# sidward14/gan-lab

Hardware: AMD Instinct MI355X
Metric: images/sec (G+D step), StyleGAN 1024^2 bs32/GPU (higher is better)
Workload: dtype f32; 1 GPU; StyleGAN res_samples=1024 FFHQ-shaped synthetic, bs=32/GPU fp32, nonsaturating + R1(lambda=10) + drift, stabilised phase, 1 D-iter + 1 G-iter; global_batch=32, per_gpu_batch=32, parallelism=single

## Files before the change

gan_lab_amd/_lib.py:

```python
import ctypes
import os
import subprocess

import torch

_HERE = os.path.dirname(os.path.abspath(__file__))
CSRC = os.path.join(_HERE, 'csrc')
SO_PATH = os.path.join(CSRC, os.path.basename(os.environ.get('GANLAB_HIP_LIB', '') or 'libganlab_hip.so'))

_c_int, _c_ll, _c_f, _c_p, _c_sz, _c_u64 = (ctypes.c_int, ctypes.c_longlong, ctypes.c_float, ctypes.c_void_p,
                                             ctypes.c_size_t, ctypes.c_uint64)

ACT_NONE, ACT_LRELU = 0, 1
PACK_FWD, PACK_DGRAD = 0, 1


class ConvGeom(ctypes.Structure):
    _fields_ = [('N', _c_int), ('Cin', _c_int), ('Hin', _c_int), ('Win', _c_int),
                ('Cout', _c_int), ('ks', _c_int), ('pad', _c_int), ('up', _c_int), ('pool', _c_int)]


_GP = ctypes.POINTER(ConvGeom)


# ... 49 lines not shown
    'ganlab_conv_s2_x3_pack': (_c_ll, [_c_p, _c_p, _c_int, _c_int, _c_int, _c_f, _c_p]),
    'ganlab_conv_s2_fwd_x3': (_c_int, [_c_p, _c_p, _c_p, _c_p, _GP, _c_f, _c_int, _c_f, _c_p]),
    'ganlab_conv_s2_fwd_aff_x3': (_c_int, [_c_p, _c_p, _c_p, _c_p, _c_p, _c_p, _GP, _c_f, _c_int, _c_f, _c_p]),
    'ganlab_conv_s2_dgrad_x3': (_c_int, [_c_p, _c_p, _c_p, _GP, _c_p]),
    'ganlab_conv_s2_down_x3_supported': (_c_int, [_GP, _c_int]),
    'ganlab_conv_s2_down_x3_pack': (_c_ll, [_c_p, _c_p, _c_int, _c_int, _c_int, _c_f, _c_p]),
    'ganlab_conv_s2_down_fwd_x3': (_c_int, [_c_p, _c_p, _c_p, _c_p, _GP, _c_f, _c_int, _c_f, _c_p]),
    'ganlab_conv_s2_down_dgrad_x3': (_c_int, [_c_p, _c_p, _c_p, _GP, _c_p]),
    'ganlab_conv_wgrad_x3_supported': (_c_int, [_GP]),
    'ganlab_conv_wgrad_x3_workspace': (_c_sz, [_GP]),
    'ganlab_conv_wgrad_x3': (_c_int, [_c_p, _c_p, _c_p, _c_p, _c_p, _GP, _c_f, _c_p, _c_sz, _c_p]),
    'ganlab_conv_s2_wgrad_x3_supported': (_c_int, [_GP]),
    'ganlab_conv_s2_wgrad_x3_workspace': (_c_sz, [_GP]),
    'ganlab_conv_s2_wgrad_x3': (_c_int, [_c_p, _c_p, _c_p, _c_p, _c_p, _GP, _c_f, _c_p, _c_sz, _c_p]),
    'ganlab_conv_fwd_aff_tail_x3': (_c_int, [_c_p, _c_p, _c_p, _c_p, _c_p, _c_p, _c_p, _c_p, _c_p, _c_p, _GP, _c_f, _c_int, _c_f,
                                             _c_f, _c_p, _c_sz, _c_p]),
    'ganlab_mask_bits_supported': (_c_int, [_c_int, _c_int]),
    'ganlab_blur3x3_bits_f32': (_c_int, [_c_p, _c_p, _c_p, _c_ll, _c_int, _c_int, _c_p]),
    'ganlab_blur_act_bwd_bits_f32': (_c_int, [_c_p, _c_p, _c_p, _c_p, _c_int, _c_int, _c_int, _c_int, _c_f, _c_f,
                                              _c_p, _c_sz, _c_p]),
    'ganlab_act_bwd_blur_bits_f32': (_c_int, [_c_p, _c_p, _c_p, _c_p, _c_p, _c_p, _c_int, _c_int, _c_int, _c_int,
                                              _c_f, _c_f, _c_p, _c_sz, _c_p]),
    'ganlab_conv_fwd_blur_supported': (_c_int, [_GP, _c_p, _c_p]),
    'ganlab_conv_fwd_blur_bits_f32': (_c_int, [_c_p, _c_p, _c_p, _c_p, _c_p, _GP, _c_f, _c_f, _c_p]),
    'ganlab_conv_s2_blur_supported': (_c_int, [_GP]),
    'ganlab_conv_s2_blur_workspace': (_c_sz, [_GP]),
    'ganlab_conv_s2_fwd_blur_tail_f32': (_c_int, [_c_p, _c_p, _c_p, _c_p, _c_p, _c_p, _c_p, _c_p, _c_p, _c_p, _GP, _c_f, _c_int,
                                                  _c_f, _c_f, _c_p, _c_sz, _c_p]),
    'ganlab_conv_s2_dgrad_blur_act_bits_f32': (_c_int, [_c_p, _c_p, _c_p, _c_p, _c_p, _GP, _c_f, _c_f, _c_p, _c_sz, _c_p]),
    'ganlab_conv_dgrad_rgb_sums_supported': (_c_int, [_GP, _c_int]),
    'ganlab_conv_dgrad_rgb_sums_workspace': (_c_sz, [_GP]),
    'ganlab_conv_dgrad_rgb_sums_f32': (_c_int, [_c_p, _c_p, _c_p, _c_p, _c_p, _c_p, _GP, _c_int, _c_f, _c_f, _c_f, _c_int, _c_int,
                                                _c_p, _c_sz, _c_p]),
    'ganlab_conv_fwd_bits_f32': (_c_int, [_c_p, _c_p, _c_p, _c_p, _c_p, _GP, _c_f, _c_int, _c_f, _c_p]),
    'ganlab_conv_dgrad_act_bits_f32': (_c_int, [_c_p, _c_p, _c_p, _c_p, _GP, _c_f, _c_p]),
    'ganlab_conv_fwd_mask_bits_f32': (_c_int, [_c_p, _c_p, _c_p, _c_p, _GP, _c_f, _c_p]),
    'ganlab_conv_wgrad_act_bits_f32': (_c_int, [_c_p, _c_p, _c_p, _c_p, _c_p, _GP, _c_f, _c_f, _c_f, _c_p, _c_sz, _c_p]),
    'ganlab_pack_desc_size': (_c_int, []),
    'ganlab_pack_many': (_c_int, [_c_p, _c_int, _c_ll, _c_p]),
    'ganlab_in_affine_f32': (_c_int, [_c_p, _c_p, _c_p, _c_p, _c_p, _c_int, _c_int, _c_p]),
    'ganlab_conv_aff_supported': (_c_int, [_GP]),
    'ganlab_conv_fwd_aff_f32': (_c_int, [_c_p, _c_p, _c_p, _c_p, _c_p, _c_p, _GP, _c_f, _c_int, _c_f, _c_p]),
    'ganlab_conv_fwd_aff_tail_chunks': (_c_int, [_GP]),
    'ganlab_conv_fwd_aff_tail_f32': (_c_int, [_c_p, _c_p, _c_p, _c_p, _c_p, _c_p, _c_p, _c_p, _c_p, _c_p, _GP, _c_f, _c_int, _c_f,
                                              _c_f, _c_p, _c_sz, _c_p]),
    'ganlab_conv_wgrad_aff_f32': (_c_int, [_c_p, _c_p, _c_p, _c_p, _c_p, _GP, _c_f, _c_p, _c_sz, _c_p]),
    'ganlab_conv_s2_aff_supported': (_c_int, [_GP]),
    'ganlab_conv_s2_fwd_aff_f32': (_c_int, [_c_p, _c_p, _c_p, _c_p, _c_p, _c_p, _GP, _c_f, _c_int, _c_f, _c_p]),
    'ganlab_conv_s2_wgrad_aff_f32': (_c_int, [_c_p, _c_p, _c_p, _c_p, _c_p, _GP, _c_f, _c_p, _c_sz, _c_p]),
    'ganlab_mod_conv_supported': (_c_int, [_GP]),
    'ganlab_mod_conv_stat_chunks': (_c_int, [_GP]),
    'ganlab_mod_conv_fwd_f32': (_c_int, [_c_p, _c_p, _c_p, _c_p, _c_p, _c_p, _c_p, _c_p, _c_p, _c_p, _GP, _c_f, _c_int,
                                         _c_f, _c_f, _c_p, _c_sz, _c_p]),
    'ganlab_mod_torgb_prep_f32': (_c_int, [_c_p, _c_p, _c_p, _c_p, _c_p, _c_p, _c_int, _c_int, _c_int, _c_f, _c_f, _c_p]),
    'ganlab_mod_torgb_wgrad_f32': (_c_int, [_c_p, _c_p, _c_p, _c_p, _c_p, _c_int, _c_int, _c_int, _c_f, _c_f, _c_p]),
    'ganlab_mod_torgb_fwd_f32': (_c_int, [_c_p, _c_p, _c_p, _c_p, _c_int, _c_int, _c_int, _c_ll, _c_p]),
    'ganlab_mod_torgb_cross_workspace': (_c_sz, [_c_int]),
    'ganlab_mod_torgb_cross_f32': (_c_int, [_c_p, _c_p, _c_p, _c_int, _c_int, _c_int, _c_ll, _c_p, _c_sz, _c_p]),
    'ganlab_blur3x3_f32': (_c_int, [_c_p, _c_p, _c_ll, _c_int, _c_int, _c_p]),
    'ganlab_up2_f32': (_c_int, [_c_p, _c_p, _c_ll, _c_int, _c_int, _c_f, _c_p]),
    'ganlab_pool2_f32': (_c_int, [_c_p, _c_p, _c_ll, _c_int, _c_int, _c_f, _c_p]),
    'ganlab_resample2d_f32': (_c_int, [_c_p, _c_p, _c_p, _c_p, _c_p, _c_p, _c_ll, _c_int, _c_int, _c_int, _c_int, _c_int,
                                       _c_int, _c_p]),
    'ganlab_bias_act_f32': (_c_int, [_c_p, _c_p, _c_p, _c_p, _c_p, _c_int, _c_int, _c_ll, _c_f, _c_int, _c_f, _c_p]),
    'ganlab_act_bwd_f32': (_c_int, [_c_p, _c_p, _c_p, _c_ll, _c_f, _c_p]),
    'ganlab_act_bwd_bias_f32': (_c_int, [_c_p, _c_p, _c_p, _c_p, _c_int, _c_int, _c_ll, _c_f, _c_f, _c_p, _c_sz, _c_p]),
# ... 152 lines not shown
```

gan_lab_amd/csrc/conv_roll_blur.hip:

```cpp
#include "common.h"

#include <stdlib.h>

namespace {

typedef unsigned int u32x4 __attribute__((ext_vector_type(4)));

constexpr int RB_TW = 64, RB_SLOTS = 6, RB_RP = 80, RB_SLOT = 16 * RB_RP, RB_Q = 18;
constexpr int RB_ITEMS = 4 * 16 * RB_Q;
constexpr int RB_PT = (RB_ITEMS + 255) / 256;
constexpr int RB_OOB = (int)0x80000000;
#ifndef RB_STORE_AUX
#define RB_STORE_AUX 0
#endif
#ifndef RB_LOAD_AUX
#define RB_LOAD_AUX 0
#endif
#ifndef RB_SETPRIO
#define RB_SETPRIO 0
#endif

struct RBArgs {
  const float* x;
  const float* wp;
  const float* bias;
  float* y;
  unsigned short* bits;
  int N, Cin, Cout, H, W;
  int Cin_p, Cout_p;
  int cols, strips, spu;
  float bias_scale, slope;
  int act;
  const float* img;
  const unsigned char* mbits;
  double* part;
  int img_c;
};
enum { RB_PLAIN = 0, RB_BLUR = 1, RB_RGB = 2 };

__device__ __forceinline__ float rb_act(float v, float slope) { return v > 0.f ? v : v * slope; }

#ifdef GL_PHASES
__device__ unsigned long long* rb_phase_buf;
#define RB_PH_DECL unsigned long long rb_t = wall_clock64(), rb_ph[10] = {0, 0, 0, 0, 0, 0, 0, 0, 0, 0};
#define RB_PH(i) { const unsigned long long rb_n = wall_clock64(); rb_ph[i] += rb_n - rb_t; rb_t = rb_n; }
#define RB_PH_FLUSH(nsteps) if (threadIdx.x == 0) { for (int i_ = 0; i_ < 10; ++i_) rb_phase_buf[(long long)blockIdx.x * 12 + i_] = rb_ph[i_]; \
    rb_phase_buf[(long long)blockIdx.x * 12 + 10] = (nsteps); rb_phase_buf[(long long)blockIdx.x * 12 + 11] = wall_clock64(); }
#else
#define RB_PH_DECL
#define RB_PH(i)
#define RB_PH_FLUSH(nsteps)
#endif

template <int MODE>
__global__ __launch_bounds__(256, MODE == RB_PLAIN ? 4 : 3) void conv_fwd_roll_blur_kernel(RBArgs p) {
  constexpr bool BLUR = MODE == RB_BLUR, RGB = MODE == RB_RGB;
  constexpr int RO = BLUR ? 1 : 0;
  __shared__ __attribute__((aligned(16))) float img_s[RGB ? 4 * 4 * 64 : 4];
  __shared__ double red_s[RGB ? 4 * 16 * 4 : 1];
  __shared__ __attribute__((aligned(16))) float ring[RB_SLOTS * RB_SLOT];
  __shared__ __attribute__((aligned(16))) float xn[2 * 4 * 16 * 4];
  __shared__ __attribute__((aligned(16))) float xe[2 * 4 * 16 * 4];
  __shared__ __attribute__((aligned(16))) unsigned bits_s[BLUR ? 16 * 8 : 4];
  __shared__ __attribute__((aligned(16))) float scratch_s[BLUR ? 256 * 4 : 4];
  const int tid = threadIdx.x, lane = tid & 63, w = tid >> 6;
  const int co = lane & 15, kk = lane >> 4;
  int bid = gl_xcd_remap(blockIdx.x, gridDim.x);
  const int txi = bid % p.cols;
  bid /= p.cols;
// ... 300 lines not shown
    }
    __syncthreads();
    if (kk == 0)
#pragma unroll
      for (int c = 0; c < 4; ++c) red_s[(w * 16 + co) * 4 + c] = rsum[c];
    __syncthreads();
    if (tid < 64 && (tid >> 2) < p.Cout) {
      const int c = tid & 3, ch = tid >> 2;
      const double t = (red_s[(0 * 16 + ch) * 4 + c] + red_s[(1 * 16 + ch) * 4 + c]) +
                       (red_s[(2 * 16 + ch) * 4 + c] + red_s[(3 * 16 + ch) * 4 + c]);
      p.part[(long long)(ch * 4 + c) * gridDim.x + blockIdx.x] = t;
    }
  }
}

__global__ void rb_rgb_finish_kernel(const double* __restrict__ part, float* __restrict__ gw, float* __restrict__ gb, int chunks,
                                     int img_c, float scale, float bias_scale, int accumulate) {
  const int ch = blockIdx.x >> 2, c = blockIdx.x & 3;
  double t = 0.0;
  for (int i = threadIdx.x; i < chunks; i += 64) t += part[(long long)blockIdx.x * chunks + i];
#pragma unroll
  for (int o = 32; o > 0; o >>= 1) t += __shfl_xor(t, o, 64);
  if (threadIdx.x != 0) return;
  if (c < img_c && gw != nullptr) {
    float* d = gw + ch * img_c + c;
    *d = ((accumulate & 1) ? *d : 0.f) + (float)(t * (double)scale);
  } else if (c == 3 && gb != nullptr) {
    gb[ch] = ((accumulate & 2) ? gb[ch] : 0.f) + (float)(t * (double)bias_scale);
  }
}

}

__global__ __launch_bounds__(256, 4) void conv_fwd_roll2_kernel(RBArgs p) {
  __shared__ __attribute__((aligned(16))) float ring[RB_SLOTS * RB_SLOT];
  constexpr int HITEMS = 2 * 16 * RB_Q, HPT = (HITEMS + 255) / 256;
  const int tid = threadIdx.x, lane = tid & 63, w = tid >> 6;
  const int co = lane & 15, kk = lane >> 4;
  int bid = gl_xcd_remap(blockIdx.x, gridDim.x);
  const int txi = bid % p.cols;
  bid /= p.cols;
  const int syi = bid % p.strips;
  const int n0 = bid / p.strips;
  const int nh = 2 * min(p.spu, p.H / 4 - syi * p.spu);
  const int ox0 = txi * RB_TW, Y0 = syi * p.spu * 4;
  const int plane = p.H * p.W;
  const float* xb = p.x + (long long)n0 * p.Cin * plane;

  int gb[HPT], lo[HPT];
#pragma unroll
  for (int i = 0; i < HPT; ++i) {
    const int e = tid + i * 256;
    const int q = e % RB_Q, t = e / RB_Q;
    const int ci = t & 15, k = t >> 4;
    const int vx = ox0 - 4 + 4 * q;
    gb[i] = (e < HITEMS && ci < p.Cin && (unsigned)vx < (unsigned)p.W) ? (ci * plane + vx) * 4 : RB_OOB;
    lo[i] = e < HITEMS ? ((ci * RB_RP + 4 * q) | (k << 16)) : -1;
  }
  float wreg[36];
#pragma unroll
  for (int st = 0; st < 36; ++st)
    wreg[st] = p.wp[(long long)((st >> 2) * p.Cin_p + (st & 3) * 4 + kk) * p.Cout_p + co];
  const bool co_ok = co < p.Cout;
  const float bv = (p.bias != nullptr && co_ok) ? p.bias[co] * p.bias_scale : 0.f;
  const long long oplane = (long long)p.H * p.W;
  const __amdgpu_buffer_rsrc_t rs_in =
      __builtin_amdgcn_make_buffer_rsrc(const_cast<float*>(xb), 0, (unsigned)(p.Cin * plane * 4), 0x00020000);
  const __amdgpu_buffer_rsrc_t rs_out = __builtin_amdgcn_make_buffer_rsrc(
      p.y + (long long)n0 * p.Cout * oplane, 0, (unsigned)(p.Cout * oplane * 4), 0x00020000);
  const int vo_lane = co_ok ? (int)(((long long)co * oplane + ox0 + w * 16 + kk * 4) * 4) : RB_OOB;
  const int W4 = p.W * 4;

  float4 xr[2][HPT];
  auto load_item = [&](int r0, bool on, int set, int i) {
    const int vy = Y0 - 1 + r0 + ((lo[i] >> 16) & 1);
    const int off = (on && gb[i] != RB_OOB && (unsigned)vy < (unsigned)p.H) ? gb[i] + vy * W4 : RB_OOB;
    const u32x4 v = __builtin_amdgcn_raw_buffer_load_b128(rs_in, off, 0, 0);
    xr[set][i] = float4{__uint_as_float(v.x), __uint_as_float(v.y), __uint_as_float(v.z), __uint_as_float(v.w)};
  };
  auto store_item = [&](int r0, int set, int i) {
    if (lo[i] != -1)
      *reinterpret_cast<float4*>(ring + ((r0 % RB_SLOTS) + ((lo[i] >> 16) & 1)) * RB_SLOT + (lo[i] & 0xffff)) = xr[set][i];
  };
#pragma unroll
  for (int i = 0; i < HPT; ++i) load_item(0, true, 0, i);
#pragma unroll
  for (int i = 0; i < HPT; ++i) load_item(2, true, 1, i);
#pragma unroll
  for (int i = 0; i < HPT; ++i) store_item(0, 0, i);
#pragma unroll
  for (int i = 0; i < HPT; ++i) store_item(2, 1, i);
#pragma unroll
  for (int i = 0; i < HPT; ++i) load_item(4, true, 0, i);
#pragma unroll
  for (int i = 0; i < HPT; ++i) load_item(6, nh > 2, 1, i);
  __syncthreads();

  f32x4 acc[2] = {f32x4{0.f, 0.f, 0.f, 0.f}, f32x4{0.f, 0.f, 0.f, 0.f}};
  const int a_lane = kk * RB_RP + w * 16 + co + 3;
  auto half_step = [&](int h, int par) {
    int sb[4];
#pragma unroll
    for (int j = 0; j < 4; ++j) sb[j] = ((2 * h + j) % RB_SLOTS) * RB_SLOT;
    constexpr int PD = 3, NF = 48;
    float rb[PD + 1];
    auto fj = [](int f) { return f < 24 ? (f & 1 ? 3 : 0) : (f < 36 ? 1 : 2); };
    auto fi = [](int f) { return f < 24 ? (f >> 1) : (f - 24) % 12; };
    auto fetch = [&](int f, int slot) {
      const int i12 = fi(f), kx = i12 >> 2, c4 = i12 & 3;
      rb[slot] = ring[sb[fj(f)] + c4 * 4 * RB_RP + kx + a_lane];
    };
    auto piece = [&](int k) {
      if (k < HPT) store_item(2 * h + 4, par, k);
      else load_item(2 * h + 8, h + 3 < nh, par, k - HPT);
    };
#pragma unroll
    for (int f = 0; f < PD; ++f) fetch(f, f % (PD + 1));
#pragma unroll
    for (int f = 0; f < NF; ++f) {
      if (f + PD < NF) fetch(f + PD, (f + PD) % (PD + 1));
      const int slot = f % (PD + 1), j = fj(f), i12 = fi(f), kx = i12 >> 2, c4 = i12 & 3;
#pragma unroll
      for (int r2 = 0; r2 < 2; ++r2) {
        const int ky = j - r2;
        if (ky >= 0 && ky < 3)
          acc[r2] = __builtin_amdgcn_mfma_f32_16x16x4f32(rb[slot], wreg[(ky * 3 + kx) * 4 + c4], acc[r2], 0, 0, 0);
      }
      if ((f & 7) == 3) {
        __builtin_amdgcn_sched_barrier(0);
        piece(f >> 3);
      }
      __builtin_amdgcn_sched_barrier(0);
    }
#pragma unroll
    for (int r2 = 0; r2 < 2; ++r2) {
      const int row = Y0 + 2 * h + r2;
      u32x4 o;
#pragma unroll
      for (int r = 0; r < 4; ++r) {
        float t = acc[r2][r] + bv;
        if (p.act == GANLAB_ACT_LRELU) t = gl_lrelu(t, p.slope);
        o[r] = __float_as_uint(t);
      }
      __builtin_amdgcn_raw_buffer_store_b128(o, rs_out, vo_lane == RB_OOB ? vo_lane : vo_lane + row * W4, 0, 0);
      acc[r2] = f32x4{0.f, 0.f, 0.f, 0.f};
    }
    __syncthreads();
  };
  for (int h = 0; h < nh; h += 2) {
    half_step(h, 0);
    half_step(h + 1, 1);
  }
}

static long long rb_plan(RBArgs& a, int N, int H, int W, int blur) {
  a.cols = W / RB_TW;
  const int steps = H / 4;
  const long long cols = (long long)a.cols * N;
  int k = 1;
  while (k < steps && cols * k < 4096 && (steps + k) / (k + 1) >= (blur ? 16 : 8)) ++k;
  a.spu = (steps + k - 1) / k;
  a.strips = (steps + a.spu - 1) / a.spu;
  return cols * a.strips;
}

bool gl_roll_blur_supported(int N, int Cin, int Cout, int H, int W, const void* x, const void* y) {
  return N > 0 && Cin >= 1 && Cin <= 16 && Cout >= 1 && Cout <= 16 && W % RB_TW == 0 && H % 4 == 0 &&
         (long long)Cin * H * W * 4 < 0x7fffffffLL && (long long)Cout * H * W * 4 < 0x7fffffffLL &&
         (reinterpret_cast<uintptr_t>(x) & 15) == 0 && (reinterpret_cast<uintptr_t>(y) & 15) == 0;
}

int gl_roll_blur_launch(const float* x, const float* wp, const float* bias, float* y, void* bits, int N, int Cin, int Cout,
                        int H, int W, int Cin_p, int Cout_p, float bias_scale, float slope, hipStream_t st, int blur,
                        int act) {
  RBArgs a{};
  a.x = x; a.wp = wp; a.bias = bias; a.y = y; a.bits = reinterpret_cast<unsigned short*>(bits);
  a.N = N; a.Cin = Cin; a.Cout = Cout; a.H = H; a.W = W; a.Cin_p = Cin_p; a.Cout_p = Cout_p;
  a.bias_scale = bias_scale; a.slope = slope; a.act = act;
  const long long grid = rb_plan(a, N, H, W, blur);
  if (grid <= 0 || grid > 0x7fffffffLL) return GANLAB_EINVAL;
  static const int half = [] { const char* e = getenv("GANLAB_ROLL_HALF"); return (e && e[0] == '0') ? 0 : 1; }();
  if (blur) GL_LAUNCH(conv_fwd_roll_blur_kernel<RB_BLUR>, dim3((unsigned)grid), dim3(256), 0, st, a);
  else if (half) GL_LAUNCH(conv_fwd_roll2_kernel, dim3((unsigned)grid), dim3(256), 0, st, a);
  else GL_LAUNCH(conv_fwd_roll_blur_kernel<RB_PLAIN>, dim3((unsigned)grid), dim3(256), 0, st, a);
  return GL_CHECK_LAUNCH();
// ... 27 lines not shown
}

size_t ganlab_conv_dgrad_rgb_sums_workspace(const ganlab_conv_geom* g) {
  if (!ganlab_conv_dgrad_rgb_sums_supported(g, 3)) return 0;
  RBArgs a{};
  const long long grid = rb_plan(a, g->N, g->Hin, g->Win, 0);
  return (size_t)g->Cin * 4 * (size_t)grid * sizeof(double);
}

int ganlab_conv_dgrad_rgb_sums_f32(const float* gy, const float* wp, const unsigned* ybits, const float* img, float* gw_rgb,
                                   float* gb_rgb, const ganlab_conv_geom* g, int img_c, float scale, float bias_scale,
                                   float slope, int acc_w, int acc_b, void* workspace, size_t workspace_bytes, void* stream) {
  if (!gy || !wp || !ybits || !img || !g || (!gw_rgb && !gb_rgb)) return GANLAB_EINVAL;
  if (!ganlab_conv_dgrad_rgb_sums_supported(g, img_c) || (reinterpret_cast<uintptr_t>(gy) & 15) ||
      (reinterpret_cast<uintptr_t>(img) & 15))
    return GANLAB_EUNSUPPORTED;
  if (!workspace || workspace_bytes < ganlab_conv_dgrad_rgb_sums_workspace(g)) return GANLAB_EWORKSPACE;
  RBArgs a{};
  a.x = gy; a.wp = wp; a.bias = nullptr; a.y = nullptr; a.bits = nullptr;
  a.N = g->N; a.Cin = g->Cout; a.Cout = g->Cin; a.H = g->Hin; a.W = g->Win;
  a.Cin_p = (g->Cout + 15) / 16 * 16; a.Cout_p = (g->Cin + 63) / 64 * 64;
  a.bias_scale = 0.f; a.slope = slope; a.act = GANLAB_ACT_NONE;
  a.img = img; a.mbits = reinterpret_cast<const unsigned char*>(ybits); a.part = reinterpret_cast<double*>(workspace);
  a.img_c = img_c;
  const long long grid = rb_plan(a, g->N, g->Hin, g->Win, 0);
  if (grid <= 0 || grid > 0x7fffffffLL) return GANLAB_EINVAL;
  hipStream_t st = gl_stream(stream);
  GL_LAUNCH(conv_fwd_roll_blur_kernel<RB_RGB>, dim3((unsigned)grid), dim3(256), 0, st, a);
  GL_LAUNCH(rb_rgb_finish_kernel, dim3((unsigned)(g->Cin * 4)), dim3(64), 0, st, (const double*)a.part, gw_rgb, gb_rgb,
            (int)grid, img_c, scale, bias_scale, (acc_w ? 1 : 0) | (acc_b ? 2 : 0));
  return GL_CHECK_LAUNCH();
}

}
```

gan_lab_amd/ops.py:

```python
import ctypes
import os

import numpy as np

import torch
from torch.autograd import Function
from torch.autograd.function import once_differentiable

from . import _lib
from ._lib import ACT_LRELU, ACT_NONE, PACK_DGRAD, PACK_FWD, ConvGeom, check


def _p(t):
    return ctypes.c_void_p(t.data_ptr()) if t is not None else None


_RAW_STREAM = getattr(torch._C, '_cuda_getCurrentRawStream', None)
_GET_DEVICE = getattr(torch._C, '_cuda_getDevice', None)


def _st():
    if _RAW_STREAM is None or _GET_DEVICE is None:
        return ctypes.c_void_p(torch.cuda.current_stream().cuda_stream)
    return ctypes.c_void_p(_RAW_STREAM(_GET_DEVICE()))
# ... 1348 lines not shown
    def forward(ctx, gy, y, x, g, s, slope, bias_scale, want_gb):
        ctx.save_for_backward(gy, y, x)
        ctx.g, ctx.s, ctx.slope = g, s, slope
        gw, gb = k_conv_wgrad_act(gy, y, x, g, s, slope, bias_scale, want_gb)
        if gb is None:
            gb = gw.new_zeros(())
            ctx.mark_non_differentiable(gb)
        return gw, gb

    @staticmethod
    def backward(ctx, ggw, ggb):
        if ggb is not None and ggb.numel() > 1 and bool(ggb.ne(0).any()):
            raise NotImplementedError('second derivative through the fused fromRGB bias gradient')
        gy, y, x = ctx.saved_tensors
        d_gy = _ConvFwdMask.apply(x, ggw, y, ctx.g, ctx.s, ctx.slope) if ctx.needs_input_grad[0] else None
        d_x = _ConvDgradAct.apply(gy, y, ggw, ctx.g, ctx.s, ctx.slope) if ctx.needs_input_grad[2] else None
        return d_gy, None, d_x, None, None, None, None, None


BLUR_HANDOFF = '_ganlab_blur_handoff'


class BlurHandoff(object):
    __slots__ = ('bits', 'slope', 'bias_scale', 'want_gb', 'gb', 'done')

    def __init__(self):
        self.bits, self.slope, self.bias_scale, self.want_gb, self.gb, self.done = None, 0.2, 1.0, False, None, False


RGB_HANDOFF = '_ganlab_rgb_handoff'


class RgbHandoff(object):
    __slots__ = ('bits', 'slope', 'img', 'w', 'bias', 'scale', 'bias_scale')

    def __init__(self):
        self.bits = None


def _rgb_fold_ok(h, g):
    import os
    if h is None or h.bits is None or torch.is_grad_enabled() or not _DIRECT[0] or not _want_param_grads() or \
            os.environ.get('GANLAB_RGB_FOLD') == '0' or get_compute_dtype() != 'f32':
        return False
    x = h.img
    if x.requires_grad and not (_NO_GRAD_TOWARDS[0] is not None and x.grad_fn is None and x.data_ptr() == _NO_GRAD_TOWARDS[0]):
        return False
    for p_ in (h.w, h.bias):
        if p_ is None:
            continue
        base = p_._base if p_._base is not None else p_
        if not base.requires_grad or getattr(base, '_ganlab_arena', None) is None or base.grad is None or \
                base.numel() != p_.numel():
            return False
    return bool(_lib.lib().ganlab_conv_dgrad_rgb_sums_supported(g.ref(), int(x.shape[1])))


def k_conv_dgrad_rgb_sums(gz, w, h, g, scale):
    gz, w = _c(gz, 'conv grad_out'), _c(w, 'conv weight')
    assert tuple(gz.shape) == g.out_shape
    _note('dgrad', g)
    L = _lib.lib()

    def slot(p_):
        base = p_._base if p_._base is not None else p_
        arena = base._ganlab_arena
        acc = getattr(base, '_ganlab_written', -1) == arena.serial
        base._ganlab_written = arena.serial
        return base.grad, int(acc)
    gw, acc_w = slot(h.w)
    gb, acc_b = slot(h.bias) if h.bias is not None else (None, 0)
    img = _c(h.img, 'image')
    ws = torch.empty((L.ganlab_conv_dgrad_rgb_sums_workspace(g.ref()) + 7) // 8, dtype=torch.float64, device=gz.device)
    check(L.ganlab_conv_dgrad_rgb_sums_f32(_p(gz), _p(_packed(w, PACK_DGRAD, scale)), h.bits.data_ptr(), _p(img), _p(gw), _p(gb),
                                           g.ref(), int(img.shape[1]), h.scale, h.bias_scale, h.slope, acc_w, acc_b,
                                           ctypes.c_void_p(ws.data_ptr()), ws.numel() * 8, _st()), 'conv_dgrad_rgb_sums')


class _ConvDgradBlurAct(Function):

    @staticmethod
    def forward(ctx, gy, w, bits, g, s, slope, bias_scale, want_gb):
        ctx.save_for_backward(gy, w, bits)
        ctx.set_materialize_grads(False)
        ctx.g, ctx.s, ctx.slope = g, s, slope
        gz, gb = k_conv_s2_dgrad_blur_act(gy, w, bits, g, s, slope, bias_scale, want_gb)
        if gb is None:
            gb = gz.new_zeros(())
            ctx.mark_non_differentiable(gb)
        return gz, gb

    @staticmethod
    def backward(ctx, gg, ggb):
        if ggb is not None:
            raise NotImplementedError('second derivative through the fused bias gradient of the blurred layer')
        gy, w, bits = ctx.saved_tensors
        if gg is None:
            return (None,) * 8
        t = _ActBwdBlur.apply(gg, bits, None, ctx.slope, 1.0, False, False)[0]
        d_gy = _ConvFwd.apply(t, w, ctx.g, ctx.s) if ctx.needs_input_grad[0] else None
        d_w = _ConvWgrad.apply(gy, t, ctx.g, ctx.s) if ctx.needs_input_grad[1] else None
        return d_gy, d_w, None, None, None, None, None, None


class _ActBwd(Function):

    @staticmethod
    def forward(ctx, gy, y, slope):
        ctx.save_for_backward(y)
        ctx.slope = slope
        return k_act_bwd(gy, y, slope)
# ... 114 lines not shown
    @staticmethod
    def backward(ctx, g):
        if ctx.has_b:
            raise NotImplementedError('double backward through the noise-weighted channel sum')
        shape = ctx.shape
        view = [1, shape[1]] + [1] * (len(shape) - 2)
        return _Scale.apply(g.view(view).expand(shape), ctx.scale), None, None, None


class _GroupBroadcast(Function):

    @staticmethod
    def forward(ctx, stat, gs, h, w):
        ctx.dims = (stat.shape[0], gs, h, w)
        G = stat.shape[0]
        return stat.view(G, 1, 1, 1, 1).expand(G, gs, 1, h, w).reshape(G * gs, 1, h, w)

    @staticmethod
    def backward(ctx, g):
        G, gs, h, w = ctx.dims
        return _ChanSum.apply(g.reshape(1, G, gs * h * w), None, 1.0), None, None, None


class _ConvBiasAct(Function):

    @staticmethod
    def forward(ctx, x, w, bias, g, s, bias_scale, act, slope, blur=False, defer=False, in_slope=None, handoff_out=None,
                handoff_in=None, rgb_out=None, rgb_in=None):
        ctx.g, ctx.s, ctx.bias_scale, ctx.act, ctx.slope, ctx.blur = g, s, bias_scale, act, slope, blur
        ctx.bias_ref = bias
        ctx.set_materialize_grads(False)
        ctx.handoff_out, ctx.handoff_in = None, handoff_in
        ctx.rgb_in = rgb_in
        if act != ACT_NONE and not blur and not defer and in_slope is None and conv_act_bwd_fusable(g) and \
                (g.Ho * g.Wo) % 32 == 0 and mask_bits_ok_plane():
            y, bits = k_conv_fwd_bits(x, w, bias, g, s, bias_scale, act, slope)
            ctx.defer, ctx.in_slope = False, None
            ctx.bias_shape = bias.shape if bias is not None else None
            ctx.save_for_backward(x, w, bits)
            if rgb_out is not None and g.ks == 1:
                rgb_out.bits, rgb_out.slope, rgb_out.img, rgb_out.w, rgb_out.bias = bits, slope, x, w, bias
                rgb_out.scale, rgb_out.bias_scale = s, bias_scale
            return y
        ctx.defer, ctx.in_slope = bool(defer), in_slope
        assert not (defer and blur)
        ctx.bias_shape = bias.shape if bias is not None else None
        if blur and act == ACT_LRELU:
            fused = k_conv_fwd_blur_bits(x, w, bias, g, s, bias_scale, slope)
            if fused is not None:
                ctx.save_for_backward(x, w, fused[1])
                ctx.handoff_out = _fill_handoff(handoff_out, fused[1], slope, bias_scale, bias)
                return fused[0]
        y = k_conv_fwd(x, w, bias, g, s, bias_scale, act, slope)
        if blur and act != ACT_NONE and mask_bits_ok(y):
            out, bits = k_blur_bits(y)
            ctx.save_for_backward(x, w, bits)
            ctx.handoff_out = _fill_handoff(handoff_out, bits, slope, bias_scale, bias)
            return out
        ctx.save_for_backward(x, w, y if (act != ACT_NONE and not defer) else None)
        return k_blur(y) if blur else y

    @staticmethod
    def backward(ctx, gy):
        if gy is None:
            return (None,) * 15
        x, w, y = ctx.saved_tensors
        params = _want_param_grads()
        want_b = ctx.bias_shape is not None and ctx.needs_input_grad[2] and params
        gb = None
        act = ACT_NONE if ctx.defer else ctx.act
        if act != ACT_NONE and not ctx.blur and ctx.in_slope is None and conv_act_bwd_fusable(ctx.g):
            gx = _ConvDgradAct.apply(gy, y, w, ctx.g, ctx.s, ctx.slope) if _wants_input_grad(ctx, x) else None
            gw = None
            if params and (ctx.needs_input_grad[1] or want_b):
                _sink('gw', w if ctx.needs_input_grad[1] else None)
                _sink('gb', ctx.bias_ref if want_b else None)
                gw, gb = _ConvWgradAct.apply(gy, y, x, ctx.g, ctx.s, ctx.slope, ctx.bias_scale, bool(want_b))
                if _sunk('gw'):
                    gw = None
                if _sunk('gb'):
                    want_b = False
            return gx, (gw if ctx.needs_input_grad[1] else None), (gb.view(ctx.bias_shape) if want_b else None), \
                None, None, None, None, None, None, None, None, None, None, None, None
        h = ctx.handoff_out
        if h is not None and h.done:
            gz, gb = gy, (h.gb if want_b else None)
            h.done, h.gb = False, None
        elif ctx.blur and act != ACT_NONE:
            _sink('gb', ctx.bias_ref if want_b else None)
            gz, gb = _BlurActBwd.apply(gy, y, ctx.slope, ctx.bias_scale, bool(want_b))
        else:
            _sink('gb', ctx.bias_ref if want_b else None)
            if ctx.blur:
                gy = _Blur.apply(gy)
            if act != ACT_NONE and want_b:
                gz, gb = _ActBwdBias.apply(gy, y, ctx.slope, ctx.bias_scale)
            else:
                gz = _ActBwd.apply(gy, y, ctx.slope) if act != ACT_NONE else gy
                if want_b:
                    gb = _ChanSum.apply(gz, None, ctx.bias_scale, 'gb')
        if _sunk('gb'):
            gb = None
        gx = None
        if _wants_input_grad(ctx, x) and ctx.in_slope is None and ctx.handoff_in is None and _rgb_fold_ok(ctx.rgb_in, ctx.g):
            k_conv_dgrad_rgb_sums(gz, w, ctx.rgb_in, ctx.g, ctx.s)
        elif _wants_input_grad(ctx, x):
            hin = ctx.handoff_in
            if hin is not None:
                gx, gba = _ConvDgradBlurAct.apply(gz, w, hin.bits, ctx.g, ctx.s, hin.slope, hin.bias_scale,
                                                  bool(hin.want_gb and params))
                hin.gb, hin.done = (gba if (hin.want_gb and params) else None), True
            else:
                gx = _ConvDgrad.apply(gz, w, ctx.g, ctx.s) if ctx.in_slope is None else \
                    _ConvDgradMask.apply(gz, w, x, ctx.g, ctx.s, ctx.in_slope)
        gw = None
        if ctx.needs_input_grad[1] and params:
            _sink('gw', w)
            gw = _ConvWgrad.apply(gz, x, ctx.g, ctx.s)
            if _sunk('gw'):
                gw = None
        return gx, gw, (gb.view(ctx.bias_shape) if want_b and gb is not None else None), None, None, None, None, \
            None, None, None, None, None, None, None, None


def _fill_handoff(h, bits, slope, bias_scale, bias):
    if h is not None:
        h.bits, h.slope, h.bias_scale = bits, slope, bias_scale
        h.want_gb = bias is not None and bias.requires_grad
        h.gb, h.done = None, False
    return h


class _BiasAct(Function):

    @staticmethod
    def forward(ctx, x, bias, noise, noise_w, bias_scale, act, slope, stats_eps=None):
        stats = None
        if stats_eps is None:
# ... 1334 lines not shown
```

include/ganlab_hip.h:

```cpp
#ifndef GANLAB_HIP_H
#define GANLAB_HIP_H

#include <stddef.h>
#include <stdint.h>

#ifdef __cplusplus
extern "C" {
#endif

#define GANLAB_OK 0
#define GANLAB_EINVAL (-1)
#define GANLAB_EWORKSPACE (-2)
#define GANLAB_ELAUNCH (-3)
#define GANLAB_EUNSUPPORTED (-4)

#define GANLAB_ACT_NONE 0
#define GANLAB_ACT_LRELU 1

#define GANLAB_PACK_FWD 0
#define GANLAB_PACK_DGRAD 1

int ganlab_abi_version(void);

int ganlab_last_launch(char* name, int cap, unsigned* grid);
// ... 258 lines not shown
                           size_t workspace_bytes, void* stream);
int ganlab_diffaug_bwd_f32(const float* gy, const float* params, float* gx, int N, int H, int W, int policy,
                           void* workspace, size_t workspace_bytes, void* stream);

int ganlab_u8_box_decode_f32(const unsigned char* in_nhwc, float* out_nchw, int N, int Hs, int Ws, int C, int factor,
                             const float* mean, const float* stdv, const unsigned char* flip, void* stream);

int ganlab_mask_bits_supported(int H, int W);
int ganlab_blur3x3_bits_f32(const float* x, float* y, unsigned* bits, long long planes, int H, int W, void* stream);
int ganlab_blur_act_bwd_bits_f32(const float* g, const unsigned* ybits, float* out, float* gb, int N, int C, int H, int W,
                                 float slope, float bias_scale, void* workspace, size_t workspace_bytes, void* stream);
int ganlab_act_bwd_blur_bits_f32(const float* g, const unsigned* ybits, const float* noise, float* out, float* gb,
                                 float* gnw, int N, int C, int H, int W, float slope, float bias_scale, void* workspace,
                                 size_t workspace_bytes, void* stream);
int ganlab_conv_fwd_bits_f32(const float* x, const float* wp, const float* bias, float* y, unsigned* ybits,
                             const ganlab_conv_geom* g, float bias_scale, int act, float slope, void* stream);
int ganlab_conv_fwd_blur_supported(const ganlab_conv_geom* g, const void* x, const void* y);
int ganlab_conv_fwd_blur_bits_f32(const float* x, const float* wp, const float* bias, float* y, unsigned* ybits,
                                  const ganlab_conv_geom* g, float bias_scale, float slope, void* stream);
int ganlab_conv_s2_blur_supported(const ganlab_conv_geom* g);
size_t ganlab_conv_s2_blur_workspace(const ganlab_conv_geom* g);
int ganlab_conv_s2_fwd_blur_tail_f32(const float* x, const float* wp, const float* aff_s, const float* aff_t,
                                     const float* bias, const float* noise, const float* noise_w, float* y, float* mean,
                                     float* rstd, const ganlab_conv_geom* g, float bias_scale, int act, float slope, float eps,
                                     void* workspace, size_t workspace_bytes, void* stream);
int ganlab_conv_s2_dgrad_blur_act_bits_f32(const float* gy, const float* wp, const unsigned* ybits, float* gz, float* gb,
                                           const ganlab_conv_geom* g, float slope, float bias_scale, void* workspace,
                                           size_t workspace_bytes, void* stream);
int ganlab_conv_dgrad_rgb_sums_supported(const ganlab_conv_geom* g, int img_c);
size_t ganlab_conv_dgrad_rgb_sums_workspace(const ganlab_conv_geom* g);
int ganlab_conv_dgrad_rgb_sums_f32(const float* gy, const float* wp, const unsigned* ybits, const float* img, float* gw_rgb,
                                   float* gb_rgb, const ganlab_conv_geom* g, int img_c, float scale, float bias_scale,
                                   float slope, int acc_w, int acc_b, void* workspace, size_t workspace_bytes, void* stream);
int ganlab_conv_dgrad_act_bits_f32(const float* gy, const unsigned* ybits, const float* wp, float* gx,
                                   const ganlab_conv_geom* g, float slope, void* stream);
int ganlab_conv_fwd_mask_bits_f32(const float* x, const float* wp, const unsigned* ybits, float* out,
                                  const ganlab_conv_geom* g, float slope, void* stream);
int ganlab_conv_wgrad_act_bits_f32(const float* gy, const unsigned* ybits, const float* x, float* gw, float* gb,
                                   const ganlab_conv_geom* g, float scale, float bias_scale, float slope, void* workspace,
                                   size_t workspace_bytes, void* stream);

#define GANLAB_PACKKIND_PLAIN 0
#define GANLAB_PACKKIND_S2 1
#define GANLAB_PACKKIND_BF16 2
#define GANLAB_PACKKIND_X3 3
typedef struct ganlab_pack_desc {
  const float* src;
  void* dst;
  int kind;
  int Cout, Cin, ks;
  int mode;
  int up;
  float scale;
  int reserved;
  long long total;
  long long block0;
} ganlab_pack_desc;
int ganlab_pack_desc_size(void);
int ganlab_pack_many(const ganlab_pack_desc* descs_device, int n_desc, long long total_blocks, void* stream);

int ganlab_in_affine_f32(const float* mean, const float* rstd, const float* style, float* s, float* t, int N, int C,
                         void* stream);
int ganlab_conv_aff_supported(const ganlab_conv_geom* g);
int ganlab_conv_fwd_aff_f32(const float* x, const float* wp, const float* aff_s, const float* aff_t, const float* bias,
                            float* y, const ganlab_conv_geom* g, float bias_scale, int act, float slope, void* stream);
int ganlab_conv_fwd_aff_tail_chunks(const ganlab_conv_geom* g);
// ... 33 lines not shown
```

Measured before the change: 167.6 images/sec.

## Fuse discriminator first-conv dgrad with fromRGB dgrad into one image-gradient kernel

Adds a templated variant of the rolling 3x3 conv kernel that, while computing the input gradient of the first discriminator conv, applies the fromRGB leaky-ReLU mask and the 1x1 fromRGB dgrad in shared memory. It writes the image gradient directly, optionally skipping the intermediate gradient tensor. This targets the R1 penalty path, where the image gradient is needed, by removing the separate dgrad-act launch and the full-resolution intermediate round trip. In exchange it adds a more complex autograd function for double-backward, extra LDS use, and a lower occupancy bound on the new kernel.

```diff
diff --git a/gan_lab_amd/_lib.py b/gan_lab_amd/_lib.py
--- a/gan_lab_amd/_lib.py
+++ b/gan_lab_amd/_lib.py
@@ -105,6 +105,8 @@
     'ganlab_conv_dgrad_rgb_sums_workspace': (_c_sz, [_GP]),
     'ganlab_conv_dgrad_rgb_sums_f32': (_c_int, [_c_p, _c_p, _c_p, _c_p, _c_p, _c_p, _GP, _c_int, _c_f, _c_f, _c_f, _c_int, _c_int,
                                                 _c_p, _c_sz, _c_p]),
+    'ganlab_conv_dgrad_rgb_img_supported': (_c_int, [_GP, _c_int]),
+    'ganlab_conv_dgrad_rgb_img_f32': (_c_int, [_c_p, _c_p, _c_p, _c_p, _c_int, _c_p, _c_p, _GP, _c_int, _c_f, _c_p]),
     'ganlab_conv_fwd_bits_f32': (_c_int, [_c_p, _c_p, _c_p, _c_p, _c_p, _GP, _c_f, _c_int, _c_f, _c_p]),
     'ganlab_conv_dgrad_act_bits_f32': (_c_int, [_c_p, _c_p, _c_p, _c_p, _GP, _c_f, _c_p]),
     'ganlab_conv_fwd_mask_bits_f32': (_c_int, [_c_p, _c_p, _c_p, _c_p, _GP, _c_f, _c_p]),
diff --git a/gan_lab_amd/csrc/conv_roll_blur.hip b/gan_lab_amd/csrc/conv_roll_blur.hip
--- a/gan_lab_amd/csrc/conv_roll_blur.hip
+++ b/gan_lab_amd/csrc/conv_roll_blur.hip
@@ -35,6 +35,9 @@
   const unsigned char* mbits;
   double* part;
   int img_c;
+  float* gimg;
+  const float* wrp;
+  int wr_cout_p;
 };
 enum { RB_PLAIN = 0, RB_BLUR = 1, RB_RGB = 2 };
 
@@ -401,8 +404,9 @@
 
 }
 
-__global__ __launch_bounds__(256, 4) void conv_fwd_roll2_kernel(RBArgs p) {
-  __shared__ __attribute__((aligned(16))) float ring[RB_SLOTS * RB_SLOT];
+constexpr int R2_XP = RB_TW + 4;
+template <bool IMG>
+__device__ __forceinline__ void conv_fwd_roll2_body(const RBArgs& p, float* ring, [[maybe_unused]] float* xch) {
   constexpr int HITEMS = 2 * 16 * RB_Q, HPT = (HITEMS + 255) / 256;
   const int tid = threadIdx.x, lane = tid & 63, w = tid >> 6;
   const int co = lane & 15, kk = lane >> 4;
@@ -435,10 +439,21 @@
   const long long oplane = (long long)p.H * p.W;
   const __amdgpu_buffer_rsrc_t rs_in =
       __builtin_amdgcn_make_buffer_rsrc(const_cast<float*>(xb), 0, (unsigned)(p.Cin * plane * 4), 0x00020000);
+  const bool store_y = !IMG || p.y != nullptr;
   const __amdgpu_buffer_rsrc_t rs_out = __builtin_amdgcn_make_buffer_rsrc(
-      p.y + (long long)n0 * p.Cout * oplane, 0, (unsigned)(p.Cout * oplane * 4), 0x00020000);
+      store_y ? p.y + (long long)n0 * p.Cout * oplane : ring, 0, store_y ? (unsigned)(p.Cout * oplane * 4) : 0u, 0x00020000);
   const int vo_lane = co_ok ? (int)(((long long)co * oplane + ox0 + w * 16 + kk * 4) * 4) : RB_OOB;
   const int W4 = p.W * 4;
+  [[maybe_unused]] float wr[16];
+  [[maybe_unused]] const int wu = __builtin_amdgcn_readfirstlane(w);
+  [[maybe_unused]] const int c_row = lane >> 5, c_px = 2 * (lane & 31);
+  if constexpr (IMG) {
+#pragma unroll
+    for (int ci = 0; ci < 16; ++ci) wr[ci] = (ci < p.Cout && wu < p.img_c) ? p.wrp[(long long)ci * p.wr_cout_p + wu] : 0.f;
+  }
+  [[maybe_unused]] const unsigned char* mbase = nullptr;
+  if constexpr (IMG)
+    mbase = p.mbits + ((((long long)n0 * p.Cout + (co_ok ? co : 0)) * p.H + Y0) * p.W + ox0 + w * 16 + kk * 4) / 8;
 
   float4 xr[2][HPT];
   auto load_item = [&](int r0, bool on, int set, int i) {
@@ -483,6 +498,11 @@
       if (k < HPT) store_item(2 * h + 4, par, k);
       else load_item(2 * h + 8, h + 3 < nh, par, k - HPT);
     };
+    [[maybe_unused]] unsigned mb[2] = {0xffu, 0xffu};
+    if constexpr (IMG) {
+#pragma unroll
+      for (int r2 = 0; r2 < 2; ++r2) mb[r2] = mbase[(2 * h + r2) * (p.W >> 3)] >> (4 * (kk & 1));
+    }
 #pragma unroll
     for (int f = 0; f < PD; ++f) fetch(f, f % (PD + 1));
 #pragma unroll
@@ -511,15 +531,49 @@
         if (p.act == GANLAB_ACT_LRELU) t = gl_lrelu(t, p.slope);
         o[r] = __float_as_uint(t);
       }
-      __builtin_amdgcn_raw_buffer_store_b128(o, rs_out, vo_lane == RB_OOB ? vo_lane : vo_lane + row * W4, 0, 0);
+      if (store_y)
+        __builtin_amdgcn_raw_buffer_store_b128(o, rs_out, vo_lane == RB_OOB ? vo_lane : vo_lane + row * W4, 0, 0);
+      if constexpr (IMG) {
+        float4 gz;
+        gz.x = (mb[r2] & 1u) ? __uint_as_float(o[0]) : __uint_as_float(o[0]) * p.slope;
+        gz.y = (mb[r2] & 2u) ? __uint_as_float(o[1]) : __uint_as_float(o[1]) * p.slope;
+        gz.z = (mb[r2] & 4u) ? __uint_as_float(o[2]) : __uint_as_float(o[2]) * p.slope;
+        gz.w = (mb[r2] & 8u) ? __uint_as_float(o[3]) : __uint_as_float(o[3]) * p.slope;
+        *reinterpret_cast<float4*>(xch + ((par * 2 + r2) * 16 + co) * R2_XP + w * 16 + kk * 4) = gz;
+      }
       acc[r2] = f32x4{0.f, 0.f, 0.f, 0.f};
     }
     __syncthreads();
+    if constexpr (IMG) {
+      if (wu < p.img_c) {
+        const float* src = xch + (par * 2 + c_row) * 16 * R2_XP + c_px;
+        float2 a = float2{0.f, 0.f};
+#pragma unroll
+        for (int ci = 0; ci < 16; ++ci) {
+          if (ci < p.Cout) {
+            const float2 v = *reinterpret_cast<const float2*>(src + ci * R2_XP);
+            a.x += wr[ci] * v.x; a.y += wr[ci] * v.y;
+          }
+        }
+        *reinterpret_cast<float2*>(p.gimg + (((long long)n0 * p.img_c + wu) * p.H + Y0 + 2 * h + c_row) * p.W + ox0 + c_px) = a;
+      }
+    }
   };
   for (int h = 0; h < nh; h += 2) {
     half_step(h, 0);
     half_step(h + 1, 1);
   }
+}
+
+__global__ __launch_bounds__(256, 4) void conv_fwd_roll2_kernel(RBArgs p) {
+  __shared__ __attribute__((aligned(16))) float ring[RB_SLOTS * RB_SLOT];
+  conv_fwd_roll2_body<false>(p, ring, nullptr);
+}
+
+__global__ __launch_bounds__(256, 3) void conv_dgrad_roll2_img_kernel(RBArgs p) {
+  __shared__ __attribute__((aligned(16))) float ring[RB_SLOTS * RB_SLOT];
+  __shared__ __attribute__((aligned(16))) float xch[2 * 2 * 16 * R2_XP];
+  conv_fwd_roll2_body<true>(p, ring, xch);
 }
 
 static long long rb_plan(RBArgs& a, int N, int H, int W, int blur) {
@@ -613,4 +667,27 @@
   return GL_CHECK_LAUNCH();
 }
 
-}
+int ganlab_conv_dgrad_rgb_img_supported(const ganlab_conv_geom* g, int img_c) {
+  return ganlab_conv_dgrad_rgb_sums_supported(g, img_c);
+}
+
+int ganlab_conv_dgrad_rgb_img_f32(const float* gy, const float* wp, const unsigned* ybits, const float* wrp, int wr_cout_p,
+                                  float* gimg, float* gx_mid, const ganlab_conv_geom* g, int img_c, float slope, void* stream) {
+  if (!gy || !wp || !ybits || !wrp || !gimg || !g || wr_cout_p < img_c) return GANLAB_EINVAL;
+  if (!ganlab_conv_dgrad_rgb_img_supported(g, img_c) || (reinterpret_cast<uintptr_t>(gy) & 15) ||
+      (reinterpret_cast<uintptr_t>(gimg) & 15) || (reinterpret_cast<uintptr_t>(gx_mid) & 15))
+    return GANLAB_EUNSUPPORTED;
+  RBArgs a{};
+  a.x = gy; a.wp = wp; a.bias = nullptr; a.y = gx_mid; a.bits = nullptr;
+  a.N = g->N; a.Cin = g->Cout; a.Cout = g->Cin; a.H = g->Hin; a.W = g->Win;
+  a.Cin_p = (g->Cout + 15) / 16 * 16; a.Cout_p = (g->Cin + 63) / 64 * 64;
+  a.bias_scale = 0.f; a.slope = slope; a.act = GANLAB_ACT_NONE;
+  a.mbits = reinterpret_cast<const unsigned char*>(ybits); a.img_c = img_c;
+  a.gimg = gimg; a.wrp = wrp; a.wr_cout_p = wr_cout_p;
+  const long long grid = rb_plan(a, g->N, g->Hin, g->Win, 0);
+  if (grid <= 0 || grid > 0x7fffffffLL) return GANLAB_EINVAL;
+  GL_LAUNCH(conv_dgrad_roll2_img_kernel, dim3((unsigned)grid), dim3(256), 0, gl_stream(stream), a);
+  return GL_CHECK_LAUNCH();
+}
+
+}
diff --git a/gan_lab_amd/ops.py b/gan_lab_amd/ops.py
--- a/gan_lab_amd/ops.py
+++ b/gan_lab_amd/ops.py
@@ -1404,10 +1404,12 @@
 
 
 class RgbHandoff(object):
-    __slots__ = ('bits', 'slope', 'img', 'w', 'bias', 'scale', 'bias_scale')
+    __slots__ = ('bits', 'slope', 'img', 'w', 'bias', 'scale', 'bias_scale', 'g', 'gimg')
 
     def __init__(self):
         self.bits = None
+        self.g = None
+        self.gimg = None
 
 
 def _rgb_fold_ok(h, g):
@@ -1449,6 +1451,63 @@
                                            ctypes.c_void_p(ws.data_ptr()), ws.numel() * 8, _st()), 'conv_dgrad_rgb_sums')
 
 
+_RGB_ONLOAD = [os.environ.get('GANLAB_RGB_ONLOAD') != '0']
+
+
+def _rgb_img_ok(h, g):
+    if h is None or h.bits is None or h.g is None or not _RGB_ONLOAD[0] or get_compute_dtype() != 'f32':
+        return False
+    x = h.img
+    if not x.requires_grad or (_NO_GRAD_TOWARDS[0] is not None and x.grad_fn is None and x.data_ptr() == _NO_GRAD_TOWARDS[0]):
+        return False
+    return g.bf is None and not g.s2 and h.g.Cout == g.Cin and \
+        bool(_lib.lib().ganlab_conv_dgrad_rgb_img_supported(g.ref(), int(x.shape[1])))
+
+
+def k_conv_dgrad_rgb_img(gz, w, bits, wr, g, scale, gr, scale_r, slope, keep_mid):
+    gz, w, wr = _c(gz, 'conv grad_out'), _c(w, 'conv weight'), _c(wr, 'fromRGB weight')
+    assert tuple(gz.shape) == g.out_shape and gr.out_shape == g.in_shape
+    _note('dgrad', g)
+    _note('dgrad', gr)
+    gimg = _new(gr.in_shape, gz)
+    mid = _new(g.in_shape, gz) if keep_mid else None
+    check(_lib.lib().ganlab_conv_dgrad_rgb_img_f32(_p(gz), _p(_packed(w, PACK_DGRAD, scale)), bits.data_ptr(),
+                                                   _p(_packed(wr, PACK_DGRAD, scale_r)), (gr.Cin + 63) // 64 * 64, _p(gimg),
+                                                   _p(mid), g.ref(), gr.Cin, slope, _st()), 'conv_dgrad_rgb_img')
+    return gimg, mid
+
+
+class _ConvDgradRgbImg(Function):
+
+    @staticmethod
+    def forward(ctx, gz, w, bits, wr, g, s, gr, sr, slope, keep_mid):
+        ctx.g, ctx.s, ctx.gr, ctx.sr, ctx.slope = g, s, gr, sr, slope
+        ctx.set_materialize_grads(False)
+        gimg, mid = k_conv_dgrad_rgb_img(gz, w, bits, wr, g, s, gr, sr, slope, keep_mid)
+        ctx.save_for_backward(gz, w, bits, wr, mid)
+        if mid is None:
+            mid = gimg.new_zeros(())
+            ctx.mark_non_differentiable(mid)
+        return gimg, mid
+
+    @staticmethod
+    def backward(ctx, gg, gmid):
+        gz, w, bits, wr, mid = ctx.saved_tensors
+        d_mid, d_wr = gmid, None
+        if gg is not None:
+            t = _ConvFwdMask.apply(gg, wr, bits, ctx.gr, ctx.sr, ctx.slope)
+            d_mid = t if d_mid is None else _Axpby.apply(t, d_mid, 1.0, 1.0)
+            if ctx.needs_input_grad[3]:
+                if mid is None or torch.is_grad_enabled():
+                    mid = _ConvDgrad.apply(gz, w, ctx.g, ctx.s)
+                d_wr = _ConvWgradAct.apply(mid, bits, gg, ctx.gr, ctx.sr, ctx.slope, 1.0, False)[0]
+        d_gz = d_w = None
+        if d_mid is not None:
+            d_gz = _ConvFwd.apply(d_mid, w, ctx.g, ctx.s) if ctx.needs_input_grad[0] else None
+            d_w = _ConvWgrad.apply(gz, d_mid, ctx.g, ctx.s) if ctx.needs_input_grad[1] else None
+        return d_gz, d_w, None, d_wr, None, None, None, None, None, None
+
+
 class _ConvDgradBlurAct(Function):
 
     @staticmethod
@@ -1629,6 +1688,7 @@
         ctx.set_materialize_grads(False)
         ctx.handoff_out, ctx.handoff_in = None, handoff_in
         ctx.rgb_in = rgb_in
+        ctx.rgb_out = None
         if act != ACT_NONE and not blur and not defer and in_slope is None and conv_act_bwd_fusable(g) and \
                 (g.Ho * g.Wo) % 32 == 0 and mask_bits_ok_plane():
             y, bits = k_conv_fwd_bits(x, w, bias, g, s, bias_scale, act, slope)
@@ -1637,7 +1697,8 @@
             ctx.save_for_backward(x, w, bits)
             if rgb_out is not None and g.ks == 1:
                 rgb_out.bits, rgb_out.slope, rgb_out.img, rgb_out.w, rgb_out.bias = bits, slope, x, w, bias
-                rgb_out.scale, rgb_out.bias_scale = s, bias_scale
+                rgb_out.scale, rgb_out.bias_scale, rgb_out.g, rgb_out.gimg = s, bias_scale, g, None
+                ctx.rgb_out = rgb_out
             return y
         ctx.defer, ctx.in_slope = bool(defer), in_slope
         assert not (defer and blur)
@@ -1659,15 +1720,21 @@
 
     @staticmethod
     def backward(ctx, gy):
+        gimg = None
+        if ctx.rgb_out is not None and ctx.rgb_out.gimg is not None:
+            gimg, ctx.rgb_out.gimg = ctx.rgb_out.gimg, None
         if gy is None:
-            return (None,) * 15
+            return (gimg,) + (None,) * 14
         x, w, y = ctx.saved_tensors
         params = _want_param_grads()
         want_b = ctx.bias_shape is not None and ctx.needs_input_grad[2] and params
         gb = None
         act = ACT_NONE if ctx.defer else ctx.act
         if act != ACT_NONE and not ctx.blur and ctx.in_slope is None and conv_act_bwd_fusable(ctx.g):
-            gx = _ConvDgradAct.apply(gy, y, w, ctx.g, ctx.s, ctx.slope) if _wants_input_grad(ctx, x) else None
+            if gimg is not None:
+                gx = gimg
+            else:
+                gx = _ConvDgradAct.apply(gy, y, w, ctx.g, ctx.s, ctx.slope) if _wants_input_grad(ctx, x) else None
             gw = None
             if params and (ctx.needs_input_grad[1] or want_b):
                 _sink('gw', w if ctx.needs_input_grad[1] else None)
@@ -1701,6 +1768,12 @@
         gx = None
         if _wants_input_grad(ctx, x) and ctx.in_slope is None and ctx.handoff_in is None and _rgb_fold_ok(ctx.rgb_in, ctx.g):
             k_conv_dgrad_rgb_sums(gz, w, ctx.rgb_in, ctx.g, ctx.s)
+        elif _wants_input_grad(ctx, x) and ctx.in_slope is None and ctx.handoff_in is None and _rgb_img_ok(ctx.rgb_in, ctx.g):
+            h = ctx.rgb_in
+            keep = torch.is_grad_enabled() or (params and any(
+                p_ is not None and p_.requires_grad for p_ in (h.w, h.bias)))
+            h.gimg, mid = _ConvDgradRgbImg.apply(gz, w, h.bits, h.w, ctx.g, ctx.s, h.g, h.scale, h.slope, keep)
+            gx = mid if keep else None
         elif _wants_input_grad(ctx, x):
             hin = ctx.handoff_in
             if hin is not None:
diff --git a/include/ganlab_hip.h b/include/ganlab_hip.h
--- a/include/ganlab_hip.h
+++ b/include/ganlab_hip.h
@@ -314,6 +314,9 @@
 int ganlab_conv_dgrad_rgb_sums_f32(const float* gy, const float* wp, const unsigned* ybits, const float* img, float* gw_rgb,
                                    float* gb_rgb, const ganlab_conv_geom* g, int img_c, float scale, float bias_scale,
                                    float slope, int acc_w, int acc_b, void* workspace, size_t workspace_bytes, void* stream);
+int ganlab_conv_dgrad_rgb_img_supported(const ganlab_conv_geom* g, int img_c);
+int ganlab_conv_dgrad_rgb_img_f32(const float* gy, const float* wp, const unsigned* ybits, const float* wrp, int wr_cout_p,
+                                  float* gimg, float* gx_mid, const ganlab_conv_geom* g, int img_c, float slope, void* stream);
 int ganlab_conv_dgrad_act_bits_f32(const float* gy, const unsigned* ybits, const float* wp, float* gx,
                                    const ganlab_conv_geom* g, float slope, void* stream);
 int ganlab_conv_fwd_mask_bits_f32(const float* x, const float* wp, const unsigned* ybits, float* out,
```

After: 168.2 images/sec, median of 3. About the same (+0.4%).
